# kcat/openal-soft

Hardware: NVIDIA H100
Metric: voice-samples/s mixed (HRTF, bsinc24, 1024-frame updates) (higher is better)
Workload: dtype f32

## Files before the change

openal-soft_b200/csrc/async_ptx.cuh:

```cuda
#pragma once
#include <cstdint>
#include <cuda_runtime.h>

namespace b200mix {

__device__ __forceinline__ uint32_t smem_u32(const void *p)
{ return static_cast<uint32_t>(__cvta_generic_to_shared(p)); }

__device__ __forceinline__ void mbar_init(uint64_t *bar, uint32_t count)
{ asm volatile("mbarrier.init.shared::cta.b64 [%0], %1;" :: "r"(smem_u32(bar)), "r"(count) : "memory"); }
__device__ __forceinline__ void mbar_fence_init()
{ asm volatile("fence.mbarrier_init.release.cluster;" ::: "memory"); }
__device__ __forceinline__ void mbar_expect_tx(uint64_t *bar, uint32_t bytes)
{ asm volatile("mbarrier.arrive.expect_tx.shared::cta.b64 _, [%0], %1;" :: "r"(smem_u32(bar)), "r"(bytes) : "memory"); }
__device__ __forceinline__ void mbar_arrive(uint64_t *bar)
{ asm volatile("mbarrier.arrive.shared::cta.b64 _, [%0];" :: "r"(smem_u32(bar)) : "memory"); }
__device__ __forceinline__ bool mbar_try_wait(uint64_t *bar, uint32_t parity)
{
    uint32_t ok;
    asm volatile("{\n\t.reg .pred p;\n\t"
                 "mbarrier.try_wait.parity.shared::cta.b64 p, [%1], %2;\n\t"
                 "selp.u32 %0, 1, 0, p;\n\t}"
                 : "=r"(ok) : "r"(smem_u32(bar)), "r"(parity) : "memory");
    return ok != 0u;
}
__device__ __forceinline__ void mbar_wait(uint64_t *bar, uint32_t parity)
{ while(!mbar_try_wait(bar, parity)) { } }

__device__ __forceinline__ void bulk_g2s(void *dst_smem, const void *src_gmem, uint32_t bytes, uint64_t *bar)
{
    asm volatile("cp.async.bulk.shared::cluster.global.mbarrier::complete_tx::bytes [%0], [%1], %2, [%3];"
        :: "r"(smem_u32(dst_smem)), "l"(src_gmem), "r"(bytes), "r"(smem_u32(bar)) : "memory");
}
__device__ __forceinline__ void fence_proxy_async_smem()
{ asm volatile("fence.proxy.async.shared::cta;" ::: "memory"); }

__device__ __forceinline__ uint64_t wgmma_smem_desc(uint32_t saddr, uint32_t lbo_bytes, uint32_t sbo_bytes)
{
    return uint64_t((saddr >> 4) & 0x3fffu) | (uint64_t((lbo_bytes >> 4) & 0x3fffu) << 16)
        | (uint64_t((sbo_bytes >> 4) & 0x3fffu) << 32);
}
__device__ __forceinline__ void wgmma_fence() { asm volatile("wgmma.fence.sync.aligned;" ::: "memory"); }
__device__ __forceinline__ void wgmma_commit() { asm volatile("wgmma.commit_group.sync.aligned;" ::: "memory"); }
template<int N> __device__ __forceinline__ void wgmma_wait()
{ asm volatile("wgmma.wait_group.sync.aligned %0;" :: "n"(N) : "memory"); }
__device__ __forceinline__ void wgmma_m64n16k8_tf32(float (&d)[8], uint64_t adesc, uint64_t bdesc, bool accumulate)
{
    asm volatile("{\n\t.reg .pred p;\n\tsetp.ne.b32 p, %10, 0;\n\t"
                 "wgmma.mma_async.sync.aligned.m64n16k8.f32.tf32.tf32 "
                 "{%0,%1,%2,%3,%4,%5,%6,%7}, %8, %9, p, 1, 1;\n\t}"
        : "+f"(d[0]), "+f"(d[1]), "+f"(d[2]), "+f"(d[3]), "+f"(d[4]), "+f"(d[5]), "+f"(d[6]), "+f"(d[7])
        : "l"(adesc), "l"(bdesc), "r"(uint32_t(accumulate)) : "memory");
}

}
```

openal-soft_b200/csrc/b200mix.cu:

```cuda
#include "../../include/b200mix.h"

#include <algorithm>
#include <cmath>
#include <cstdio>
#include <cstdlib>
#include <cstring>
#include <new>
#include <string>
#include <vector>

#include <cuda_runtime.h>

#include <dlfcn.h>

#include "mixer_kernels.cuh"
#include "effect_kernels.cuh"
#include "shard_kernels.cuh"
#include "panmix_tc.cuh"
#include "param_kernels.hpp"
#include "efx_kernels.hpp"
#include "resampler_tables.hpp"
#include "hrtf_store.hpp"
#include "adpcm.hpp"
#include "callback_plan.hpp"
// ... 3 lines not shown

namespace {

thread_local std::string g_create_error;

}

struct b200mix_device {
    b200mix_device_desc desc{};
    int cuda_dev{0};
    int num_sms{0};
    cudaStream_t stream{nullptr};
    std::string error;
    uint64_t launches{0};

    BsincTable bsinc[3];
    DevArray<float> d_bsinc[3], d_cubic[2];

    DevArray<VoiceRec> d_voices; DevArray<BufferRec> d_buffers;
    std::vector<BufferRec> h_buffers;
    std::vector<DevArray<char>> buf_store;
    std::vector<uint32_t> h_vbuf;
    std::vector<uint32_t> h_bufrefs;
    DevArray<float2> d_hrtf_tgt, d_hrtf_old;
    DevArray<float> d_dry_cur, d_dry_tgt, d_send_cur, d_send_tgt;
    VoiceResult *d_results{nullptr};
    b200mix_voice_result *h_results{nullptr};
    DevArray<char> d_outblock; PinnedArray<char> h_outblock; size_t out_real_bytes{0};

    uint32_t dry_alloc_ch{0};
    DevArray<float> d_dry, d_wet;
    float *d_real{nullptr};
    DevArray<float> d_partial; size_t partial_floats{0};
    DevArray<float> d_accum_sum;
    DevArray<float> d_carry[2];
    int carry_idx{0};
    float *h_real{nullptr};

    uint32_t dec_channels{0}, dec_ir{0};
    DevArray<float2> d_dec_coef; DevArray<float> d_dec_hfscale, d_dec_state;
    DevArray<float> d_temp, d_temp2;
    uint32_t amb_in{0}; bool amb_dual{false};
    DevArray<float> d_amb_hf, d_amb_lf, d_amb_state;
    bool dry_active{false};
    DevArray<float> d_uhj_state, d_uhj_scratch;
    uint32_t stab_center{B200MIX_NO_SLOT};
    float stab_coeff{0.0f};
    DevArray<float> d_stab_state;
    uint32_t bs2b_level{0};
    DevArray<float> d_bs2b;
    uint32_t uhj_fir{0};
    DevArray<float> d_uhj_fir_state, d_uhj_fir_coef;

    UploadArena stage;

    std::vector<SlotRec> h_slots;
    DevArray<SlotRec> d_slots;
    std::vector<std::vector<DevArray<char>>> slot_allocs;
    uint32_t active_slots{0};
    DevArray<float> d_xscratch; DevArray<uint32_t> d_sendinfo;
    DevArray<FilterRec> d_filt;
    UploadArena fstage;
    DevArray<float> d_fscratch, d_dline;
    std::vector<uint8_t> h_dfilt;
    std::vector<uint32_t> h_order2;
    DevArray<uint32_t> d_order2;
    uint32_t num_order2{0};
// ... 57 lines not shown
    std::vector<uint32_t> h_order;
    DevArray<uint32_t> d_order;
    uint32_t num_order{0};
    bool order_dirty{true};

    UploadArena src;
    bool dev_filters{false};
    bool panmix_tc{false};

    struct Shard {
        uint32_t rank{0}, world{1}; int transport{0};
        DevArray<char> own;
        char *peer[kShardMaxWorld]{};
        size_t off_real{0}, off_wet{0}, real_floats{0}, wet_src_floats{0};
        uint32_t owned_max{0};
        uint32_t epoch{0};
        DevArray<uint32_t> d_counters;
        PinnedArray<uint32_t> h_status;
        Event ev[4];
        bool ev_wet{false}, ev_real{false};
        void *nccl_lib{nullptr}; void *comm{nullptr};
        int (*reduce)(const void*, void*, size_t, int, int, int, void*, cudaStream_t){nullptr};
        int (*allreduce)(const void*, void*, size_t, int, int, void*, cudaStream_t){nullptr};
        int (*comm_destroy)(void*){nullptr};
    } shard;

    uint32_t ir_pad{0};
    uint32_t voice_hi{0};
    void (*mix_fn)(const MixParams){nullptr};
    size_t mix_smem{0}; int mix_cdr{0}; int mix_blocks_per_sm{1};
    uint32_t reverb_seq{0};
    DevArray<uint32_t> d_claim;
    int fir_blocks_per_sm{0};

    struct CbBuf {
        bool used{false};
        uint32_t buffer{0};
        b200mix_callback_buffer cb{};
        cbplan::State st{};
        uint32_t frame_bytes{0};
    };
    std::vector<CbBuf> cbs;
    std::vector<int32_t> cb_of_buffer;
    struct CbVoice { int32_t slot{-1}; cbplan::Voice v{}; };
    std::vector<CbVoice> cbv;
    uint32_t cb_bound{0};
    UploadArena cb_arena[2]; int cb_idx{0};
    DevArray<char> d_cb_zero;
    std::vector<int32_t> cb_reps;
    std::vector<std::vector<uint32_t>> cb_members;
    struct CbWork { cbplan::State start; cbplan::Loads loads; size_t region{0}, bytes{0}; };
    std::vector<CbWork> cb_work;
    ~b200mix_device() { if(stream) cudaStreamDestroy(stream); }
};

namespace {
constexpr uint32_t kCbMaxChannels = 16;
constexpr size_t kCbPad = 256;
}

namespace {

#define CUDA_TRY(dev, expr) do { cudaError_t e_ = (expr); if(e_ != cudaSuccess) {            \
    (dev)->error = std::string(#expr) + ": " + cudaGetErrorString(e_); return B200MIX_ERR_CUDA; } } while(0)

template<typename T>
int upload(b200mix_device *d, DevArray<T> &dst, const std::vector<T> &src)
{
    if(!src.empty())
        CUDA_TRY(d, cudaMemcpyAsync(dst.get(), src.data(), src.size()*sizeof(T), cudaMemcpyHostToDevice, d->stream));
    CUDA_TRY(d, cudaStreamSynchronize(d->stream));
    return B200MIX_OK;
}

using MixKernel = void(*)(const MixParams);

struct FirVariant { MixKernel fn; size_t smem; };
FirVariant get_fir(uint32_t ir_size)
{
    if(ir_size <= 64u)
        return FirVariant{k_hrtf_fir<17, 64>, sizeof(FirSmem<kFirGS, 17, 64>)*kFirGroups};
    return FirVariant{k_hrtf_fir<19, 128>, sizeof(FirSmem<kFirGS, 19, 128>)*kFirGroups};
}

constexpr uint32_t kDryChunksMax = 128;

int ensure_park_lines(b200mix_device *d)
{
    if(d->d_xscratch) return B200MIX_OK;
    const uint32_t nv = d->desc.max_voices;
    DevArray<float> xscratch; DevArray<uint32_t> sendinfo;
    CUDA_TRY(d, xscratch.alloc(size_t(nv)*kLine, d->stream));
    CUDA_TRY(d, sendinfo.alloc(nv, d->stream));
    d->d_xscratch = std::move(xscratch); d->d_sendinfo = std::move(sendinfo);
    return B200MIX_OK;
}

int ensure_dry_park(b200mix_device *d)
{
    const b200mix_device_desc &dd = d->desc;
    if(d->d_dry_entries) return B200MIX_OK;
    if(int rc = ensure_park_lines(d)) return rc;
    if(dd.dry_channels > 4u && dd.dry_channels <= uint32_t(kPmN))
    {
        CUDA_TRY(d, cudaFuncSetAttribute(k_panmix_tc, cudaFuncAttributeMaxDynamicSharedMemorySize,
            kPmStages*kPmStageBytes + 1024));
        const char *simt = std::getenv("B200MIX_PANMIX_SIMT");
        d->panmix_tc = !(simt && simt[0] == '1');
    }
    DevArray<SendEntry> entries; DevArray<uint32_t> slotStart;
    DevArray<float> partial, geff; DevArray<float4> gramp;
    CUDA_TRY(d, entries.alloc(dd.max_voices, d->stream));
    CUDA_TRY(d, slotStart.alloc(2, d->stream));
    CUDA_TRY(d, partial.alloc(size_t(kDryChunksMax)*dd.dry_channels*kLine, d->stream));
    CUDA_TRY(d, geff.alloc(size_t(dd.max_voices)*dd.dry_channels, d->stream));
    CUDA_TRY(d, gramp.alloc(size_t(dd.max_voices)*dd.dry_channels, d->stream));
    d->d_dry_entries = std::move(entries); d->d_dry_slot_start = std::move(slotStart);
// ... 154 lines not shown
        {
            if(int rc = ensure_park_lines(d)) return rc;
            CUDA_TRY(d, d->d_claim.alloc(2, d->stream));
        }
        if(hrtfDev)
        {
            const FirVariant fir = get_fir(dd.ir_size);
            CUDA_TRY(d, cudaFuncSetAttribute(fir.fn, cudaFuncAttributeMaxDynamicSharedMemorySize, int(fir.smem)));
            CUDA_TRY(d, cudaOccupancyMaxActiveBlocksPerMultiprocessor(&perSm, fir.fn, kFirGS*kFirGroups, fir.smem));
            d->fir_blocks_per_sm = std::max(std::min(perSm, kFirCtasPerSm), 1);
        }

        d->dry_alloc_ch = std::max<uint32_t>(std::max(dd.dry_channels, 1u), uint32_t(d->mix_cdr));
        CUDA_TRY(d, d->d_dry.alloc(size_t(d->dry_alloc_ch)*kLine, d->stream));
        {
            const size_t realFloats = size_t(std::max(dd.real_channels, 1u))*kLine;
            static_assert(sizeof(VoiceResult) == 16 && sizeof(b200mix_voice_result) == 16, "result layout");
            const size_t blockBytes = realFloats*sizeof(float) + size_t(dd.max_voices)*sizeof(VoiceResult);
            CUDA_TRY(d, d->d_outblock.alloc(blockBytes, d->stream));
            char *blk = d->d_outblock;
            d->d_results = reinterpret_cast<VoiceResult*>(blk + realFloats*sizeof(float));
            CUDA_TRY(d, d->h_outblock.alloc(blockBytes));
            d->h_real = reinterpret_cast<float*>(d->h_outblock.get());
            d->h_results = reinterpret_cast<b200mix_voice_result*>(d->h_outblock + realFloats*sizeof(float));
            d->out_real_bytes = realFloats*sizeof(float);
            if(dd.post_process == B200MIX_POST_NONE) d->d_real = d->d_dry;
            else d->d_real = reinterpret_cast<float*>(blk);
        }
        if(dd.max_slots && dd.wet_channels)
            CUDA_TRY(d, d->d_wet.alloc(size_t(dd.max_slots)*dd.wet_channels*kLine, d->stream));
        d->partial_floats = hrtfDev ? size_t(d->num_sms)*d->fir_blocks_per_sm*(2*kAccumLen)
            : size_t(d->num_sms)*d->mix_blocks_per_sm*size_t(d->mix_cdr)*kLine;
        CUDA_TRY(d, d->d_partial.alloc(std::max<size_t>((hrtfDev ? 1 : 2)*d->partial_floats, 4), d->stream));
        CUDA_TRY(d, d->d_accum_sum.alloc(2*kAccumLen, d->stream));
        CUDA_TRY(d, d->d_carry[0].alloc(2*kHrirLen, d->stream));
        CUDA_TRY(d, d->d_carry[1].alloc(2*kHrirLen, d->stream));
        CUDA_TRY(d, d->d_temp.alloc(size_t(std::max(dd.dry_channels, 1u))*kLine, d->stream));
        CUDA_TRY(d, d->d_temp2.alloc(size_t(std::max(dd.dry_channels, 1u))*kLine, d->stream));
        if(dd.max_slots && dd.wet_channels && dd.num_sends)
        {
            d->h_slots.assign(dd.max_slots, SlotRec{});
            d->slot_allocs.resize(dd.max_slots);
            CUDA_TRY(d, d->d_slots.alloc(dd.max_slots, d->stream));
            if(int rc = ensure_park_lines(d)) return rc;
            CUDA_TRY(d, d->d_send_geff.alloc(size_t(dd.max_voices)*dd.num_sends*dd.wet_channels, d->stream));
            CUDA_TRY(d, d->d_send_gramp.alloc(size_t(dd.max_voices)*dd.num_sends*dd.wet_channels, d->stream));
            d->h_send_slot.assign(size_t(dd.max_voices)*B200MIX_MAX_SENDS, B200MIX_NO_SLOT);
            CUDA_TRY(d, d->d_slot_start.alloc(dd.max_slots + 1, d->stream));
            CUDA_TRY(d, d->d_entries.alloc(size_t(dd.max_voices)*dd.num_sends, d->stream));
            std::vector<float2> tw(128);
            for(int k = 0;k < 128;++k)
            {
                const double a = -2.0*3.14159265358979323846*double(k)/256.0;
                tw[k] = make_float2(float(std::cos(a)), float(std::sin(a)));
            }
            const std::vector<float> cf = BuildCubicFilter();
            CUDA_TRY(d, d->d_cubic_filter.alloc(cf.size()));
            if(int rc = upload(d, d->d_cubic_filter, cf)) return rc;
            CUDA_TRY(d, d->d_twiddle.alloc(tw.size()));
            if(int rc = upload(d, d->d_twiddle, tw)) return rc;
        }
        if(dd.post_process == B200MIX_POST_UHJ || dd.post_process == B200MIX_POST_TSME)
        {
            CUDA_TRY(d, d->d_uhj_state.alloc(64, d->stream));
            CUDA_TRY(d, d->d_uhj_scratch.alloc(5*1025, d->stream));
        }
        if(int rc = ensure_stage(d, std::min(dd.max_voices, 4096u))) return rc;
// ... 1338 lines not shown
        for(uint32_t v : d->h_order) if(d->dev_filters || d->h_dfilt[v]) d->h_order2.push_back(v);
        d->num_order2 = uint32_t(d->h_order2.size());
        if(d->num_order2)
            if(int rc = upload(d, d->d_order2, d->h_order2)) return rc;
        d->order2_dirty = false;
    }
    const bool hrtfDev = dd.ir_size > 0;
    const uint32_t nv = std::max(d->voice_hi, 1u);
    const uint32_t maxBlocks = uint32_t(d->num_sms*d->mix_blocks_per_sm);
    const uint32_t blocks = std::max(1u, std::min(maxBlocks, (d->num_order + kMixGroups - 1)/kMixGroups));

    MixParams P{};
    P.voices = d->d_voices; P.buffers = d->d_buffers;
    P.hrtf_tgt = d->d_hrtf_tgt; P.hrtf_old = d->d_hrtf_old;
    P.dry_cur = d->d_dry_cur; P.dry_tgt = d->d_dry_tgt;
    P.partial = d->d_partial;
    P.results = want_results ? d->d_results : nullptr;
    for(int i = 0;i < 3;++i) P.bsinc_tab[i] = d->d_bsinc[i];
    for(int i = 0;i < 2;++i) P.cubic_tab[i] = d->d_cubic[i];
    P.max_voices = nv; P.frames = frames; P.ir_pad = d->ir_pad;
    P.cd = dd.dry_channels; P.num_sends = dd.num_sends;
    P.order = d->d_order; P.num_order = d->num_order;
    P.xscratch = d->d_xscratch; P.sendinfo = d->d_sendinfo;
    P.filt = d->d_filt; P.filt_paths = 1u + dd.num_sends;
    P.qhdr = d->d_qhdr; P.queue = d->d_queue;
    P.claim = d->d_claim;
    P.dline = d->d_dline;
    P.cbplan = cbplan;
    stage_mark(d, 1);
    if(d->profile) cudaEventRecord(d->ev_mix0, d->stream);
    d->mix_fn<<<blocks, kMixGS*kMixGroups, d->mix_smem, d->stream>>>(P);
    ++d->launches;
    CUDA_TRY(d, cudaGetLastError());

    stage_mark(d, 2);
    size_t rows2 = 0;
    if(d->d_filt && d->num_order2)
    {
        FilterRunParams FP{};
        FP.filt = d->d_filt; FP.filt_paths = 1u + dd.num_sends; FP.sendinfo = d->d_sendinfo;
        FP.direct_order = d->d_order2; FP.num_direct = d->num_order2;
        FP.xscratch = d->d_xscratch; FP.dline = d->d_dline; FP.frames = frames;
        k_filters<<<(d->num_order2 + 31u)/32u, 32, 0, d->stream>>>(FP);
        ++d->launches;
        if(d->mix_cdr > 0)
        {
            const uint32_t blocks2 = std::max(1u, std::min(maxBlocks, (d->num_order2 + kMixGroups - 1)/kMixGroups));
            rows2 = blocks2;
            MixParams P2 = P;
            P2.order = d->d_order2; P2.num_order = d->num_order2;
            P2.partial = d->d_partial + d->partial_floats;
            P2.results = nullptr;
            k_mix_deferred<kMixGS, kMixGroups, 4><<<blocks2, kMixGS*kMixGroups,
                sizeof(DeferredSmem<kMixGroups, 4>), d->stream>>>(P2);
            ++d->launches;
        }
        CUDA_TRY(d, cudaGetLastError());
    }
    uint32_t firBlocks = 0;
    if(hrtfDev)
    {
        const FirVariant fir = get_fir(dd.ir_size);
        firBlocks = std::max(1u, std::min(uint32_t(d->num_sms*d->fir_blocks_per_sm),
            (d->num_order + kFirGroups - 1)/kFirGroups));
        fir.fn<<<firBlocks, kFirGS*kFirGroups, fir.smem, d->stream>>>(P);
        ++d->launches;
        CUDA_TRY(d, cudaGetLastError());
    }
    if(d->profile) { cudaEventRecord(d->ev_mix1, d->stream); d->ev_valid = true; }

    stage_mark(d, 3);
    if(hrtfDev)
    {
        const uint32_t len = 2*kAccumLen;
        k_reduce_rows<<<(len/4 + kReduceCols - 1)/kReduceCols, 1024, 0, d->stream>>>(d->d_partial, firBlocks, len,
            d->d_accum_sum, 0);
        ++d->launches;
    }
    if(d->mix_cdr > 0)
    {
        const uint32_t len = uint32_t(d->mix_cdr)*kLine;
        k_reduce_rows<<<(len/4 + kReduceCols - 1)/kReduceCols, 1024, 0, d->stream>>>(d->d_partial, blocks, len, d->d_dry, 1);
        ++d->launches;
        if(rows2)
        {
            k_reduce_rows<<<(len/4 + kReduceCols - 1)/kReduceCols, 1024, 0, d->stream>>>(d->d_partial + d->partial_floats,
                uint32_t(rows2), len, d->d_dry, 1);
            ++d->launches;
        }
    }
    CUDA_TRY(d, cudaGetLastError());

    stage_mark(d, 4);
    if(d->mix_cdr == 0 && d->d_dry_entries)
    {
        if(d->dry_entries_dirty)
        {
            d->h_dry_entries.clear();
            for(uint32_t v = 0;v < d->voice_hi;++v)
                if(d->h_active[v] && !d->h_hrtf[v]) d->h_dry_entries.push_back(SendEntry{v, 0u});
            d->num_dry_entries = uint32_t(d->h_dry_entries.size());
            const uint32_t ss[2] = {0u, d->num_dry_entries};
            CUDA_TRY(d, cudaMemcpyAsync(d->d_dry_slot_start, ss, sizeof(ss), cudaMemcpyHostToDevice, d->stream));
            if(int rc = upload(d, d->d_dry_entries, d->h_dry_entries)) return rc;
            d->dry_entries_dirty = false;
        }
        if(d->num_dry_entries)
        {
            SendMixParams DM{};
            DM.slot_start = d->d_dry_slot_start; DM.entries = d->d_dry_entries; DM.sendinfo = d->d_sendinfo;
            DM.xscratch = d->d_xscratch; DM.send_cur = d->d_dry_cur; DM.send_tgt = d->d_dry_tgt;
// ... 152 lines not shown
            }
            if(convWork)
            {
                k_conv_input<<<dd.max_slots, 128, 0, d->stream>>>(CP);
                k_conv_mac<<<dim3(dd.max_slots, convCh, CP.chunks), 128, sizeof(ConvMacSmem), d->stream>>>(CP);
                k_conv_ifft<<<dim3(dd.max_slots, convCh, kConvMaxBlocks), 128, 0, d->stream>>>(CP);
                k_conv_output<<<dim3(dd.max_slots, convCh), 128, 0, d->stream>>>(CP);
                d->launches += 4;
            }
            k_slot_output_mix<<<dim3((frames + 127)/128, dd.dry_channels), 128, 0, d->stream>>>(SP);
            ++d->launches;
            if(d->any_target)
            {
                k_slot_target_mix<<<dim3((frames + 127)/128, dd.max_slots), 128, 0, d->stream>>>(SP);
                ++d->launches;
            }
        }
        k_slot_gains_commit<<<dd.max_slots, 64, 0, d->stream>>>(SP);
        ++d->launches;
        for(auto &eh : d->efx)
        {
            if(eh.used && eh.p.type == B200MIX_EFFECT_MODULATOR) eh.mod_index = (eh.mod_index + frames) % eh.mod_range;
            if(eh.used && eh.p.type == B200MIX_EFFECT_CHORUS) eh.lfo_offset = (eh.lfo_offset + frames) % eh.lfo_range;
        }
        CUDA_TRY(d, cudaGetLastError());
    }

    stage_mark(d, 7);
    switch(dd.post_process)
    {
    case B200MIX_POST_HRTF:
    {
        PostHrtfParams Q{};
        Q.accum_sum = d->d_accum_sum; Q.carry_in = d->d_carry[d->carry_idx];
        Q.carry_out = d->d_carry[d->carry_idx^1];
        Q.dry = d->d_dry; Q.real = d->d_real; Q.dec_coef = d->d_dec_coef;
        Q.dec_hfscale = d->d_dec_hfscale; Q.dec_state = d->d_dec_state; Q.temp = d->d_temp;
        Q.frames = frames; Q.cd = dd.dry_channels; Q.dec_ir = d->dec_ir;
        Q.real_left = dd.real_left; Q.real_right = dd.real_right; Q.dry_active = d->dry_active;
        if(d->dry_active)
        {
            k_post_hrtf_split<<<dd.dry_channels, 32, 0, d->stream>>>(Q);
            ++d->launches;
        }
        Q.overwrite = d->real_overwrite ? 1u : 0u;
        k_post_hrtf_mix<<<dim3((frames + kHrirLen + 127)/128, 2), 128, 0, d->stream>>>(Q);
        ++d->launches;
        d->carry_idx ^= 1;
        break;
    }
    case B200MIX_POST_AMBIDEC:
    {
        PostAmbiParams Q{};
        Q.dry = d->d_dry; Q.real = d->d_real; Q.gains_hf = d->d_amb_hf; Q.gains_lf = d->d_amb_lf;
        Q.split_state = d->d_amb_state; Q.temp_hf = d->d_temp; Q.temp_lf = d->d_temp2;
        Q.frames = frames; Q.cd = dd.dry_channels; Q.real_channels = dd.real_channels;
        Q.dual = d->amb_dual;
        if(d->amb_dual)
        {
            k_post_ambi_split<<<1, 32, 0, d->stream>>>(Q);
            ++d->launches;
        }
        const uint32_t total = dd.real_channels*frames;
        k_post_ambi_mix<<<(total + 127)/128, 128, 0, d->stream>>>(Q);
        ++d->launches;
        if(d->stab_center != B200MIX_NO_SLOT)
        {
            StabParams S{};
            S.real = d->d_real; S.state = d->d_stab_state; S.frames = frames;
            S.real_channels = dd.real_channels; S.lidx = dd.real_left; S.ridx = dd.real_right;
            S.cidx = d->stab_center; S.coeff = d->stab_coeff;
            const float halfPi = 3.14159265358979323846f*0.5f;
            S.mid_lf = std::cos(1.0f/3.0f * halfPi); S.mid_hf = std::cos(1.0f/4.0f * halfPi);
            S.center_lf = std::sin(1.0f/3.0f * halfPi); S.center_hf = std::sin(1.0f/4.0f * halfPi);
            const size_t smem = size_t(2u + dd.real_channels)*kLine*sizeof(float);
            k_post_stabilizer<<<1, 32u*dd.real_channels, smem, d->stream>>>(S);
            ++d->launches;
        }
        else if(d->bs2b_level)
        {
// ... 29 lines not shown
}

static int render_output_stage(b200mix_device *d, uint32_t frames)
{
    const b200mix_device_desc &dd = d->desc;
    if(d->shard.transport && d->shard.rank != 0u) return B200MIX_OK;
    if(d->d_limiter)
    {
        LimiterParams LQ{d->d_limiter, d->d_real, d->d_limiter_delay, frames};
        k_limiter<<<1, 1024, 0, d->stream>>>(LQ);
        ++d->launches;
    }
    if(d->d_dc_delay)
    {
        DistCompParams DQ{d->d_real, d->d_dc_buf, d->d_dc_delay, d->d_dc_gain, frames};
        k_distance_comp<<<dd.real_channels, 1024, 0, d->stream>>>(DQ);
        ++d->launches;
    }
    CUDA_TRY(d, cudaGetLastError());
    return B200MIX_OK;
}

static int shard_wet_exchange(b200mix_device *d)
{
    b200mix_device::Shard &S = d->shard;
    const b200mix_device_desc &dd = d->desc;
    if(!S.transport || !d->d_wet) return B200MIX_OK;
    if(d->profile) { cudaEventRecord(S.ev[0], d->stream); }
    const size_t wetFloats = size_t(dd.max_slots)*dd.wet_channels*kLine;
    if(S.transport == 2)
    {
        if(S.allreduce(d->d_wet, d->d_wet, wetFloats, 7 , 0 , S.comm, d->stream) != 0)
        { d->error = "ncclAllReduce of the wet buffers failed"; return B200MIX_ERR_CUDA; }
    }
    else
    {
        const uint32_t slotFloats = dd.wet_channels*uint32_t(kLine);
        ShardPushParams P{};
        P.src = d->d_wet; P.rank = S.rank; P.world = S.world; P.epoch = S.epoch;
        P.wet = 1u; P.num_slots = dd.max_slots; P.slot_floats = slotFloats; P.owned_max = S.owned_max;
        P.own = reinterpret_cast<ShardCtl*>(S.own.get());
        for(uint32_t r = 0;r < S.world;++r) P.peer[r] = S.peer[r];
        P.off_data = S.off_wet; P.per_src_floats = S.wet_src_floats;
        P.counters = S.d_counters + 4;
        const uint32_t chunks = std::max(1u, std::min(32u, slotFloats*S.owned_max/(4u*256u*4u)));
        k_shard_push<<<dim3(chunks, S.world), 256, 0, d->stream>>>(P);
        ShardSumParams Q{};
        Q.dst = d->d_wet; Q.rank = S.rank; Q.world = S.world; Q.epoch = S.epoch;
        Q.wet = 1u; Q.num_slots = dd.max_slots; Q.slot_floats = slotFloats; Q.owned_max = S.owned_max;
        Q.own = P.own; for(uint32_t r = 0;r < S.world;++r) Q.peer[r] = S.peer[r];
        Q.off_data = S.off_wet; Q.per_src_floats = S.wet_src_floats; Q.counter = S.d_counters + 2;
        k_shard_sum<<<std::max(1u, std::min(64u, slotFloats*S.owned_max/(4u*256u*2u))), 256, 0, d->stream>>>(Q);
        d->launches += 2;
        CUDA_TRY(d, cudaGetLastError());
    }
    if(d->profile) { cudaEventRecord(S.ev[1], d->stream); S.ev_wet = true; }
    return B200MIX_OK;
}

static int shard_real_reduce(b200mix_device *d)
{
    b200mix_device::Shard &S = d->shard;
    const b200mix_device_desc &dd = d->desc;
    if(!S.transport) return B200MIX_OK;
    if(d->profile) { cudaEventRecord(S.ev[2], d->stream); }
    const uint32_t floats = dd.real_channels*uint32_t(kLine);
// ... 280 lines not shown
        || (dither_depth > 0.0f && !dither_seed))
    { d->error = "render_interleaved: bad arguments"; return B200MIX_ERR_INVALID; }
    if(int rc = render_launch(d, frames, results != nullptr)) return rc;
    static const size_t sz[] = {1, 1, 2, 2, 4, 4, 4};
    if(!d->h_outbuf)
    {
        CUDA_TRY(d, d->d_outbuf.alloc(size_t(kLine)*64*4));
        CUDA_TRY(d, d->h_outbuf.alloc(size_t(kLine)*64*4));
    }
    OutputParams Q{};
    Q.real = d->d_real; Q.out = d->d_outbuf; Q.frames = frames; Q.channels = dd.real_channels;
    Q.frame_step = frame_step; Q.out_type = out_type; Q.dither_depth = dither_depth;
    Q.seed = dither_seed ? *dither_seed : 0u;
    const uint32_t total = frames*frame_step;
    k_output_write<<<(total + 255)/256, 256, 0, d->stream>>>(Q);
    ++d->launches;
    CUDA_TRY(d, cudaGetLastError());
    const size_t bytes = size_t(total)*sz[out_type];
    CUDA_TRY(d, cudaMemcpyAsync(d->h_outbuf, d->d_outbuf, bytes, cudaMemcpyDeviceToHost, d->stream));
    if(int rc = render_collect(d, frames, nullptr, results)) return rc;
    std::memcpy(out, d->h_outbuf, bytes);
    if(dither_depth > 0.0f) *dither_seed = lcg_skip_host(*dither_seed, uint64_t(2)*dd.real_channels*frames);
    return B200MIX_OK;
}

int b200mix_render_begin(b200mix_device *d, uint32_t frames, float **wet_dev, size_t *wet_floats)
{
    if(!d) return B200MIX_ERR_INVALID;
    if(d->mid_render) { d->error = "render_begin: already begun"; return B200MIX_ERR_INVALID; }
    if(d->shard.transport)
    { d->error = "render_begin: a sharded device set exchanges its wet buffers itself — use b200mix_render"; return B200MIX_ERR_INVALID; }
    if(int rc = render_phase_a(d, frames, true, true)) return rc;
    d->mid_render = true; d->mid_frames = frames;
    if(wet_dev) *wet_dev = d->d_wet;
    if(wet_floats) *wet_floats = d->d_wet ? size_t(d->desc.max_slots)*d->desc.wet_channels*kLine : 0;
    return B200MIX_OK;
}

int b200mix_render_end(b200mix_device *d, float *const *real_out, b200mix_voice_result *results,
    const float **real_out_dev)
{
    if(!d) return B200MIX_ERR_INVALID;
    if(!d->mid_render) { d->error = "render_end: no render_begin pending"; return B200MIX_ERR_INVALID; }
    d->mid_render = false;
    if(int rc = render_phase_b(d, d->mid_frames)) return rc;
    if(int rc = render_output_stage(d, d->mid_frames)) return rc;
    if(real_out_dev) *real_out_dev = d->d_real;
    if(!real_out && !results) return B200MIX_OK;
    return render_collect(d, d->mid_frames, real_out, results);
}

int b200mix_render_device(b200mix_device *d, uint32_t frames, const float **real_out_dev)
{
    if(!d) return B200MIX_ERR_INVALID;
    if(int rc = render_launch(d, frames, false)) return rc;
    if(real_out_dev) *real_out_dev = d->d_real;
    return B200MIX_OK;
}

static void shard_release(b200mix_device *d)
{
    b200mix_device::Shard &S = d->shard;
    if(S.transport == 1)
        for(uint32_t r = 0;r < S.world;++r)
            if(r != S.rank && S.peer[r]) cudaIpcCloseMemHandle(S.peer[r]);
    if(S.comm && S.comm_destroy) S.comm_destroy(S.comm);
// ... 212 lines not shown
```

openal-soft_b200/csrc/mixer_kernels.cuh:

```cuda
#pragma once
#include <cstddef>
#include <cstdint>
#include <cuda_runtime.h>

#include "voice_structs.hpp"
#include "async_ptx.cuh"

namespace b200mix {

constexpr int kLine = 1024;
constexpr int kHrirLen = 128;
constexpr int kHist = 64;
constexpr int kEdge = 24;
constexpr int kPad = 48;
constexpr int kResBuf = kLine + 256 + kPad;
constexpr int kSrcSizeMax = kResBuf - kEdge;
constexpr int kAccumLen = kLine + kHrirLen;
constexpr float kSilence = 0.00001f;
constexpr float kEps = 1.1920929e-07f;

constexpr uint32_t kVfStatic = 1u<<2, kVfLooping = 1u<<3, kVfHrtf = 1u<<4;
constexpr uint32_t kVfFading = 1u<<8, kVfHaveBuffer = 1u<<9, kVfCoefDirty = 1u<<10;
constexpr uint32_t kUpNoBuffer = 1u<<11;
constexpr uint32_t kVfChannelMask = 0xffu<<16;
// ... 1015 lines not shown
                }
                group_sync(bar, GS);

                if(pack && winInt && !packedWin)
                {
                    pack_window16<GS>(S.win, srcn, t, bar);
                    packedWin = true;
                }
                resample_chunk<GS>(S.win, S.tabF, S.tabD, xs, loaded, dstn, increment, fracPos,
                    resampler, m, tapOff, ms, packedWin, t);
            }
            advance_chunk<GS>(S.win, rec.prev, packedWin, silent, playing, n, loaded, dstn, increment,
                fracPos, intPos, t, bar);
        }
        group_sync(bar, GS);

        const uint32_t counter = (flags & kVfFading) ? (n < 64u ? n : 64u) : 0u;
        if(P.sendinfo)
            park_voice<GS, CDR>(P, xs, v, rec.send_mask, defer, isHrtf, playing, dirty, counter, t);
        if(dfilt && !defer) filter_clear(*dfilt, t);
        if constexpr(CDR > 0)
            if(!defer)
                mix_dry<GS, CDR>(accD, xs, S.newGain, P.dry_cur + size_t(v)*P.cd, P.dry_tgt + size_t(v)*P.cd,
                    P.cd, n, counter, playing, t);
        if(t == 0)
            write_back_voice(P, rec, v, h1, flags, vstate, increment, haveBuffer, isQueue, qh, qitems,
                looping, loopStart, loopEnd, buf.frames);
        group_sync(bar, GS);
        if(CDR > 0 && !defer) store_dry_gains(P.dry_cur + size_t(v)*P.cd, S.newGain, P.cd, t);
        group_sync(bar, GS);
    }

    if constexpr(CDR > 0) store_partial_row<GS, GROUPS, CDR>(accD, smem_raw, P.partial, g, t);
}

template<int GROUPS, int CDR>
union DeferredSmem {
    struct { float x[kLine]; float newGain[32]; } group[GROUPS];
    float stage[CDR*kLine];
};

template<int GS, int GROUPS, int CDR>
__global__ void __launch_bounds__(GS*GROUPS)
k_mix_deferred(const MixParams P)
{
    extern __shared__ __align__(16) unsigned char smem_raw[];
    const int g = threadIdx.x / GS;
    const int t = threadIdx.x % GS;
    auto &S = reinterpret_cast<DeferredSmem<GROUPS, CDR>*>(smem_raw)->group[g];
    const int bar = 1 + g;
    constexpr int SPT = kLine / GS;

    float accD[CDR][SPT];
    #pragma unroll
    for(int c = 0;c < CDR;++c)
        #pragma unroll
        for(int r = 0;r < SPT;++r) accD[c][r] = 0.0f;

    const uint32_t n = P.frames;
    const uint32_t groups = gridDim.x*GROUPS;
    for(uint32_t oi = blockIdx.x*GROUPS + g;oi < P.num_order;oi += groups)
    {
        const uint32_t v = P.order[oi];
        const uint32_t info = P.sendinfo[v];
        if(!(info & kSiDeferred)) continue;
        const float *fl = P.dline + size_t(v)*kLine;
// ... 28 lines not shown
    const uint32_t lineBytes = (n & ~3u)*4u, irBytes = P.ir_pad*8u;
    const bool dirty = (info & kSiDirty) != 0;
    const float *line = ((info & kSiDeferred) ? P.dline : P.xscratch) + size_t(v)*kLine;
    fence_proxy_async_smem();
    mbar_expect_tx(bar, kHist*4u + lineBytes + (dirty ? 2u : 1u)*irBytes);
    bulk_g2s(B.x, P.voices[v].hist, kHist*4u, bar);
    if(lineBytes) bulk_g2s(B.x + kHist, line, lineBytes, bar);
    bulk_g2s(B.coefT, P.hrtf_tgt + size_t(v)*P.ir_pad, irBytes, bar);
    if(dirty) bulk_g2s(B.coefO, P.hrtf_old + size_t(v)*P.ir_pad, irBytes, bar);
}

template<int OPT, int FP>
__global__ void __launch_bounds__(kFirGS*kFirGroups, kFirCtasPerSm)
k_hrtf_fir(const MixParams P)
{
    constexpr int GS = kFirGS, GROUPS = kFirGroups;
    using Smem = FirSmem<GS, OPT, FP>;
    extern __shared__ __align__(16) unsigned char smem_raw[];
    const int g = threadIdx.x / GS;
    const int t = threadIdx.x % GS;
    Smem &S = reinterpret_cast<Smem*>(smem_raw)[g];
    const int bar = 1 + g;
    const int t0 = OPT*t;
    const uint32_t n = P.frames;

    float2 acc[OPT];
    #pragma unroll
    for(int r = 0;r < OPT;++r) acc[r] = make_float2(0.0f, 0.0f);

    for(int i = t;i < FP;i += GS) S.lLR[i] = make_float2(0.0f, 0.0f);
    for(int i = FP + int(n) + t;i < Smem::kLLen;i += GS) S.lLR[i] = make_float2(0.0f, 0.0f);
    if(t == 0) { mbar_init(&S.bar[0], 1u); mbar_init(&S.bar[1], 1u); mbar_fence_init(); }
    group_sync(bar, GS);

    const uint32_t stride = gridDim.x*GROUPS;
    uint32_t v = 0u, info = 0u;
    uint32_t oi = next_hrtf_voice(P, blockIdx.x*GROUPS + g, stride, v, info);
    if(t == 0 && oi < P.num_order) fir_stage_issue(P, S.st[0], &S.bar[0], v, info, n);
    uint32_t parity = 0u;
    for(int b = 0;oi < P.num_order;b ^= 1)
    {
        VoiceRec &rec = P.voices[v];
        const uint4 *hp = reinterpret_cast<const uint4*>(&rec);
        const uint4 h3 = hp[3], h4 = hp[4];

        uint32_t vN = 0u, infoN = 0u;
        const uint32_t oiN = next_hrtf_voice(P, oi + stride, stride, vN, infoN);
        if(t == 0 && oiN < P.num_order) fir_stage_issue(P, S.st[b^1], &S.bar[b^1], vN, infoN, n);

        FirStage &B = S.st[b];
        const bool playing = (info & kSiPlaying) != 0;
        const bool dirty = (info & kSiDirty) != 0;
        const uint32_t counter = (info >> 8) & 0xffu;

        const float *line = ((info & kSiDeferred) ? P.dline : P.xscratch) + size_t(v)*kLine;
        for(uint32_t k = (n & ~3u) + t;k < n;k += GS) B.x[kHist + k] = line[k];
        mbar_wait(&S.bar[b], (parity >> b) & 1u);
        parity ^= 1u << b;
        if(n & 3u) group_sync(bar, GS);

        if(playing)
            for(int k = t;k < kHist;k += GS) rec.hist[k] = B.x[n + k];
        uint32_t oD0 = h4.x, oD1 = h4.y;
        float oGain = __uint_as_float(h4.z);
        const uint32_t tD0 = h3.y, tD1 = h3.z;
        const float tgtGain = __uint_as_float(h3.w);
// ... 38 lines not shown
            in[s] = make_float2(xl[s] * gnew, xr[s] * gnew);
        }
        const bool oldPass = !sameFilter && oldOn;
        if(oldPass)
            for(int i = t;i < Smem::kOLen;i += GS)
            {
                const int s = i - FP;
                float l = 0.0f, r = 0.0f;
                if(s >= 0 && uint32_t(s) < fademix)
                {
                    const float gold = oldStep*float(fademix - uint32_t(s));
                    l = hs[kHist - oD0 + s] * gold;
                    r = hs[kHist - oD1 + s] * gold;
                }
                S.oLR[i] = make_float2(l, r);
            }
        group_sync(bar, GS);

        const int irpad = int(P.ir_pad);
        fir_pass<OPT, FP>(acc, S.lLR, B.coefT, irpad, t0);
        if(oldPass && t0 < int(kHist) + irpad)
            fir_pass<OPT, FP>(acc, S.oLR, dirty ? B.coefO : B.coefT, irpad, t0);
        if(t == 0)
        {
            rec.old_delay0 = tD0; rec.old_delay1 = tD1;
            rec.old_gain = targetGain;
        }
        group_sync(bar, GS);
        oi = oiN; v = vN; info = infoN;
    }

    const size_t row = blockIdx.x;
    __syncthreads();
    float *stage = reinterpret_cast<float*>(smem_raw);
    for(int gg = 0;gg < GROUPS;++gg)
    {
        if(g == gg)
        {
            #pragma unroll
            for(int r = 0;r < OPT;++r)
            {
                const int o = t0 + r;
                if(o < kAccumLen)
                {
                    if(gg == 0) { stage[o] = acc[r].x; stage[kAccumLen + o] = acc[r].y; }
                    else { stage[o] += acc[r].x; stage[kAccumLen + o] += acc[r].y; }
                }
            }
            if(gg == 0 && GS*OPT < kAccumLen)
                for(int o = GS*OPT + t;o < kAccumLen;o += GS) { stage[o] = 0.0f; stage[kAccumLen + o] = 0.0f; }
        }
        __syncthreads();
    }
    float *pl = P.partial + row*(2*kAccumLen);
    for(int o = threadIdx.x;o < 2*kAccumLen;o += GS*GROUPS) pl[o] = stage[o];
}


constexpr int kReduceCols = 8, kReduceSegs = 128;
__global__ void __launch_bounds__(1024)
k_reduce_rows(const float *__restrict__ partial, uint32_t rows, uint32_t len,
    float *__restrict__ out, int accumulate)
{
    __shared__ float4 sm[kReduceSegs][kReduceCols];
    const uint32_t col = threadIdx.x & (kReduceCols-1), seg = threadIdx.x / kReduceCols;
    const uint32_t e4 = blockIdx.x*kReduceCols + col;
    float4 s = make_float4(0.f, 0.f, 0.f, 0.f);
    if(e4*4u < len)
    {
        const uint32_t per = (rows + kReduceSegs - 1u)/kReduceSegs;
        const uint32_t r0 = seg*per, r1 = (r0 + per < rows) ? r0 + per : rows;
        const float4 *p = reinterpret_cast<const float4*>(partial) + e4;
        const size_t stride4 = len/4u;
        uint32_t r = r0;
        for(;r + 4u <= r1;r += 4u)
        {
            const float4 a = __ldg(p + size_t(r)*stride4), b = __ldg(p + size_t(r+1)*stride4);
            const float4 c = __ldg(p + size_t(r+2)*stride4), d = __ldg(p + size_t(r+3)*stride4);
            s.x += a.x; s.y += a.y; s.z += a.z; s.w += a.w;
            s.x += b.x; s.y += b.y; s.z += b.z; s.w += b.w;
            s.x += c.x; s.y += c.y; s.z += c.z; s.w += c.w;
            s.x += d.x; s.y += d.y; s.z += d.z; s.w += d.w;
        }
        for(;r < r1;++r)
        {
            const float4 a = __ldg(p + size_t(r)*stride4);
            s.x += a.x; s.y += a.y; s.z += a.z; s.w += a.w;
        }
    }
    sm[seg][col] = s;
    __syncthreads();
    #pragma unroll
    for(uint32_t width = kReduceSegs/4u;width >= 1u;width /= 4u)
    {
        float4 tot = make_float4(0.f, 0.f, 0.f, 0.f);
        const bool on = seg < width;
        if(on)
        {
            tot = sm[seg*4u][col];
            #pragma unroll
            for(uint32_t k = 1;k < 4u;++k)
            {
                const float4 a = sm[seg*4u + k][col];
                tot.x += a.x; tot.y += a.y; tot.z += a.z; tot.w += a.w;
            }
        }
        __syncthreads();
        if(on) sm[seg][col] = tot;
        __syncthreads();
        if(width == 2u) break;
    }
    if(seg == 0 && e4*4u < len)
    {
        float4 tot = sm[0][col];
        const float4 b = sm[1][col];
        tot.x += b.x; tot.y += b.y; tot.z += b.z; tot.w += b.w;
        float4 *o = reinterpret_cast<float4*>(out) + e4;
        if(accumulate)
        {
            const float4 a = *o;
            tot.x += a.x; tot.y += a.y; tot.z += a.z; tot.w += a.w;
        }
        *o = tot;
    }
}

__global__ void __launch_bounds__(256)
k_reduce_few(const float *__restrict__ partial, uint32_t rows, uint32_t len,
    float *__restrict__ out, int accumulate)
{
    const uint32_t e4 = blockIdx.x*blockDim.x + threadIdx.x;
    if(e4*4u >= len) return;
    const float4 *p = reinterpret_cast<const float4*>(partial) + e4;
    const size_t stride4 = len/4u;
    float4 v[16];
    #pragma unroll
    for(uint32_t r = 0;r < 16u;++r)
        v[r] = r < rows ? __ldg(p + size_t(r)*stride4) : make_float4(0.f, 0.f, 0.f, 0.f);
    float4 g[4];
    #pragma unroll
    for(uint32_t j = 0;j < 4u;++j)
    {
        float4 t = v[4u*j];
        #pragma unroll
        for(uint32_t k = 1;k < 4u;++k)
        { t.x += v[4u*j+k].x; t.y += v[4u*j+k].y; t.z += v[4u*j+k].z; t.w += v[4u*j+k].w; }
        g[j] = t;
    }
    float4 tot = g[0];
// ... 216 lines not shown
            fl |= kVfHaveBuffer;
            if(up.flags & (1u<<6)) fl |= kVfFading;
            rec.old_delay0 = 0; rec.old_delay1 = 0; rec.old_gain = 0.0f;
            if(A.qhdr) A.qhdr[up.voice].y = 0u;
        }
        else
        {
            fl |= oldFlags & (kVfFading|kVfHaveBuffer|kVfCoefDirty);
        }
        if(up.has_coeffs && !reset) fl |= kVfCoefDirty;
        if(up.flags & kUpNoBuffer) fl &= ~kVfHaveBuffer;
        rec.flags = fl;
        if(up.flags & (1u<<7)) rec.state = 0u;
        else if(up.flags & (1u<<1)) rec.state = 2u;
        else if(up.flags & (1u<<0)) rec.state = 1u;
        rec.buffer = up.buffer; rec.resampler = up.resampler;
        rec.loop_start = up.loop_start; rec.loop_end = up.loop_end; rec.step = up.step;
        rec.bsinc_sf = up.bsinc_sf; rec.bsinc_m = up.bsinc_m; rec.bsinc_l = up.bsinc_l;
        rec.bsinc_off = up.bsinc_off;
        rec.tgt_delay0 = fromDirs ? sB.delay[0] : up.delay0;
        rec.tgt_delay1 = fromDirs ? sB.delay[1] : up.delay1;
        rec.tgt_gain = up.gain;
        uint32_t mask = 0;
        for(int s = 0;s < kMaxSends;++s)
        {
            rec.send_slot[s] = up.send_slot[s];
            if(up.send_slot[s] != 0xffffffffu) mask |= 1u<<s;
        }
        rec.send_mask = mask;
    }
}

struct PostHrtfParams {
    const float *accum_sum;
    const float *carry_in;
    float *carry_out;
    const float *dry;
    float *real;
    const float2 *dec_coef;
    const float *dec_hfscale; float *dec_state;
    float *temp;
    uint32_t frames, cd, dec_ir, real_left, real_right, dry_active;
    uint32_t overwrite;
};

__global__ void __launch_bounds__(32) k_post_hrtf_split(const PostHrtfParams Q)
{
    __shared__ float line[kLine];
    const uint32_t c = blockIdx.x;
    if(c >= Q.cd) return;
    const uint32_t lane = threadIdx.x, n = Q.frames;
    const float *in = Q.dry + size_t(c)*kLine;
    float *out = Q.temp + size_t(c)*kLine;
    for(uint32_t i = lane;i < kLine;i += 32) line[i] = (i < n) ? in[i] : 0.0f;
    __syncwarp();
    if(lane == 0)
    {
        float *st = Q.dec_state + c*4;
        const float ap_coeff = st[0];
        const float lp_coeff = st[0]*0.5f + 0.5f;
        float lp_z1 = st[1], lp_z2 = st[2], ap_z1 = st[3];
        const float hfscale = Q.dec_hfscale[c];
        for(uint32_t i0 = 0;i0 < n;i0 += 8)
        {
            float x[8], y[8];
            #pragma unroll
            for(int k = 0;k < 8;++k) x[k] = line[i0+k];
            #pragma unroll
            for(int k = 0;k < 8;++k)
            {
                const float d0 = (x[k] - lp_z1) * lp_coeff;
                const float lp_y0 = lp_z1 + d0;
                const float nz1 = lp_y0 + d0*lp_coeff;
                const float d1 = (lp_y0 - lp_z2) * lp_coeff;
                const float lp_y1 = lp_z2 + d1;
                const float nz2 = lp_y1 + d1;
                const float ap_y = x[k]*ap_coeff + ap_z1;
                const float naz = x[k] - ap_y*ap_coeff;
                y[k] = (ap_y-lp_y1)*hfscale + lp_y1;
                if(i0 + k < n) { lp_z1 = nz1; lp_z2 = nz2; ap_z1 = naz; }
            }
            #pragma unroll
            for(int k = 0;k < 8;++k) line[i0+k] = y[k];
        }
        st[1] = lp_z1; st[2] = lp_z2; st[3] = ap_z1;
    }
    __syncwarp();
    for(uint32_t i = lane;i < n;i += 32) out[i] = line[i];
}

__global__ void __launch_bounds__(128) k_post_hrtf_mix(const PostHrtfParams Q)
{
    __shared__ float xs[128 + kHrirLen];
    __shared__ float cf[kHrirLen];
    const uint32_t span = Q.frames + kHrirLen;
    const uint32_t ear = blockIdx.y;
    const uint32_t t0 = blockIdx.x*128u, tt = t0 + threadIdx.x;
    float tot = 0.0f;
    if(tt < span)
    {
        tot = Q.accum_sum[ear*kAccumLen + tt];
        if(tt < uint32_t(kHrirLen)) tot += Q.carry_in[ear*kHrirLen + tt];
    }
    if(Q.dry_active)
    {
        const uint32_t jmax = Q.dec_ir;
        for(uint32_t c = 0;c < Q.cd;++c)
        {
            const float *x = Q.temp + size_t(c)*kLine;
            const float2 *cg = Q.dec_coef + size_t(c)*Q.dec_ir;
            __syncthreads();
            for(uint32_t k = threadIdx.x;k < 128u + kHrirLen;k += 128u)
            {
                const int src = int(t0) - int(kHrirLen) + int(k);
                xs[k] = (src >= 0 && src < int(Q.frames)) ? x[src] : 0.0f;
            }
            if(threadIdx.x < jmax) cf[threadIdx.x] = ear ? cg[threadIdx.x].y : cg[threadIdx.x].x;
            __syncthreads();
            float s = 0.0f;
            const float *w = xs + kHrirLen + threadIdx.x;
            for(uint32_t j = 0;j < jmax;++j)
                s = fmaf(cf[j], w[-int(j)], s);
            tot += s;
        }
    }
    if(tt >= span) return;
    if(tt < Q.frames)
    {
        float *o = Q.real + size_t(ear ? Q.real_right : Q.real_left)*kLine + tt;
        *o = Q.overwrite ? tot : (*o + tot);
    }
    else
        Q.carry_out[ear*kHrirLen + (tt - Q.frames)] = tot;
}

struct PostAmbiParams {
    const float *dry; float *real; const float *gains_hf; const float *gains_lf;
    float *split_state; float *temp_hf; float *temp_lf;
    uint32_t frames, cd, real_channels, dual;
};

__global__ void k_post_ambi_split(const PostAmbiParams Q)
{
    const uint32_t c = blockIdx.x*blockDim.x + threadIdx.x;
    if(c >= Q.cd) return;
    float *st = Q.split_state + c*4;
    const float ap_coeff = st[0];
    const float lp_coeff = st[0]*0.5f + 0.5f;
    float lp_z1 = st[1], lp_z2 = st[2], ap_z1 = st[3];
    const float *in = Q.dry + size_t(c)*kLine;
    float *hp = Q.temp_hf + size_t(c)*kLine, *lp = Q.temp_lf + size_t(c)*kLine;
    for(uint32_t i = 0;i < Q.frames;++i)
    {
        const float x = in[i];
        const float d0 = (x - lp_z1) * lp_coeff;
        const float lp_y0 = lp_z1 + d0;
        lp_z1 = lp_y0 + d0;
        const float d1 = (lp_y0 - lp_z2) * lp_coeff;
        const float lp_y1 = lp_z2 + d1;
        lp_z2 = lp_y1 + d1;
        lp[i] = lp_y1;
        const float ap_y = x*ap_coeff + ap_z1;
        ap_z1 = x - ap_y*ap_coeff;
// ... 677 lines not shown
```

Baseline: 31.06 billion.

## Fuse HRTF partial-row reduction into post-HRTF mix and chain kernels with PDL

Removes the separate k_reduce_rows launch and the accum_sum buffer by having a new k_post_hrtf_reduce kernel sum FIR partial rows per 32-sample tile, then add the carry and the per-channel decoder FIR, with one thread per (dry channel, output). Adds programmatic dependent launch (griddepcontrol) between the mix, FIR and post kernels so each can start its prologue before the previous one finishes. The reduce loop is also batched eight rows at a time to keep more loads in flight. In exchange, many more blocks each re-read decoder coefficients and input, and the post kernel is limited to 32 dry channels.

After: 32.29 billion, median of 6. 1.04x the previous value.

```diff
diff --git a/openal-soft_b200/csrc/async_ptx.cuh b/openal-soft_b200/csrc/async_ptx.cuh
--- a/openal-soft_b200/csrc/async_ptx.cuh
+++ b/openal-soft_b200/csrc/async_ptx.cuh
@@ -35,6 +35,10 @@
 __device__ __forceinline__ void fence_proxy_async_smem()
 { asm volatile("fence.proxy.async.shared::cta;" ::: "memory"); }
 
+__device__ __forceinline__ void griddep_wait() { asm volatile("griddepcontrol.wait;" ::: "memory"); }
+__device__ __forceinline__ void griddep_launch_dependents()
+{ asm volatile("griddepcontrol.launch_dependents;" ::: "memory"); }
+
 __device__ __forceinline__ uint64_t wgmma_smem_desc(uint32_t saddr, uint32_t lbo_bytes, uint32_t sbo_bytes)
 {
     return uint64_t((saddr >> 4) & 0x3fffu) | (uint64_t((lbo_bytes >> 4) & 0x3fffu) << 16)
diff --git a/openal-soft_b200/csrc/b200mix.cu b/openal-soft_b200/csrc/b200mix.cu
--- a/openal-soft_b200/csrc/b200mix.cu
+++ b/openal-soft_b200/csrc/b200mix.cu
@@ -59,7 +59,7 @@
     DevArray<float> d_dry, d_wet;
     float *d_real{nullptr};
     DevArray<float> d_partial; size_t partial_floats{0};
-    DevArray<float> d_accum_sum;
+    uint32_t fir_rows{0};
     DevArray<float> d_carry[2];
     int carry_idx{0};
     float *h_real{nullptr};
@@ -183,6 +183,7 @@
     uint32_t reverb_seq{0};
     DevArray<uint32_t> d_claim;
     int fir_blocks_per_sm{0};
+    uint64_t fir_done{0};
 
     struct CbBuf {
         bool used{false};
@@ -234,6 +235,22 @@
     return FirVariant{k_hrtf_fir<19, 128>, sizeof(FirSmem<kFirGS, 19, 128>)*kFirGroups};
 }
 
+static_assert(kPostMaxDry == B200MIX_MAX_DRY_CHANNELS, "k_post_hrtf_reduce: one thread per dry channel");
+
+template<typename... Args>
+cudaError_t launch_ex(b200mix_device *d, bool programmatic, void (*fn)(Args...), dim3 grid, dim3 block,
+    size_t smem, Args... args)
+{
+    cudaLaunchAttribute attr{};
+    attr.id = cudaLaunchAttributeProgrammaticStreamSerialization;
+    attr.val.programmaticStreamSerializationAllowed = 1;
+    cudaLaunchConfig_t cfg{};
+    cfg.gridDim = grid; cfg.blockDim = block; cfg.dynamicSmemBytes = smem; cfg.stream = d->stream;
+    cfg.attrs = programmatic ? &attr : nullptr; cfg.numAttrs = programmatic ? 1u : 0u;
+    ++d->launches;
+    return cudaLaunchKernelEx(&cfg, fn, args...);
+}
+
 constexpr uint32_t kDryChunksMax = 128;
 
 int ensure_park_lines(b200mix_device *d)
@@ -454,7 +471,6 @@
         d->partial_floats = hrtfDev ? size_t(d->num_sms)*d->fir_blocks_per_sm*(2*kAccumLen)
             : size_t(d->num_sms)*d->mix_blocks_per_sm*size_t(d->mix_cdr)*kLine;
         CUDA_TRY(d, d->d_partial.alloc(std::max<size_t>((hrtfDev ? 1 : 2)*d->partial_floats, 4), d->stream));
-        CUDA_TRY(d, d->d_accum_sum.alloc(2*kAccumLen, d->stream));
         CUDA_TRY(d, d->d_carry[0].alloc(2*kHrirLen, d->stream));
         CUDA_TRY(d, d->d_carry[1].alloc(2*kHrirLen, d->stream));
         CUDA_TRY(d, d->d_temp.alloc(size_t(std::max(dd.dry_channels, 1u))*kLine, d->stream));
@@ -1859,6 +1875,7 @@
     d->mix_fn<<<blocks, kMixGS*kMixGroups, d->mix_smem, d->stream>>>(P);
     ++d->launches;
     CUDA_TRY(d, cudaGetLastError());
+    const uint64_t mixDone = d->launches;
 
     stage_mark(d, 2);
     size_t rows2 = 0;
@@ -1884,26 +1901,19 @@
         }
         CUDA_TRY(d, cudaGetLastError());
     }
-    uint32_t firBlocks = 0;
+    d->fir_rows = 0;
     if(hrtfDev)
     {
         const FirVariant fir = get_fir(dd.ir_size);
-        firBlocks = std::max(1u, std::min(uint32_t(d->num_sms*d->fir_blocks_per_sm),
+        d->fir_rows = std::max(1u, std::min(uint32_t(d->num_sms*d->fir_blocks_per_sm),
             (d->num_order + kFirGroups - 1)/kFirGroups));
-        fir.fn<<<firBlocks, kFirGS*kFirGroups, fir.smem, d->stream>>>(P);
-        ++d->launches;
-        CUDA_TRY(d, cudaGetLastError());
+        CUDA_TRY(d, launch_ex(d, d->launches == mixDone, fir.fn, dim3(d->fir_rows), dim3(kFirGS*kFirGroups),
+            fir.smem, P));
+        d->fir_done = d->launches;
     }
     if(d->profile) { cudaEventRecord(d->ev_mix1, d->stream); d->ev_valid = true; }
 
     stage_mark(d, 3);
-    if(hrtfDev)
-    {
-        const uint32_t len = 2*kAccumLen;
-        k_reduce_rows<<<(len/4 + kReduceCols - 1)/kReduceCols, 1024, 0, d->stream>>>(d->d_partial, firBlocks, len,
-            d->d_accum_sum, 0);
-        ++d->launches;
-    }
     if(d->mix_cdr > 0)
     {
         const uint32_t len = uint32_t(d->mix_cdr)*kLine;
@@ -2122,7 +2132,7 @@
     case B200MIX_POST_HRTF:
     {
         PostHrtfParams Q{};
-        Q.accum_sum = d->d_accum_sum; Q.carry_in = d->d_carry[d->carry_idx];
+        Q.partial = d->d_partial; Q.rows = d->fir_rows; Q.carry_in = d->d_carry[d->carry_idx];
         Q.carry_out = d->d_carry[d->carry_idx^1];
         Q.dry = d->d_dry; Q.real = d->d_real; Q.dec_coef = d->d_dec_coef;
         Q.dec_hfscale = d->d_dec_hfscale; Q.dec_state = d->d_dec_state; Q.temp = d->d_temp;
@@ -2134,8 +2144,8 @@
             ++d->launches;
         }
         Q.overwrite = d->real_overwrite ? 1u : 0u;
-        k_post_hrtf_mix<<<dim3((frames + kHrirLen + 127)/128, 2), 128, 0, d->stream>>>(Q);
-        ++d->launches;
+        CUDA_TRY(d, launch_ex(d, d->launches == d->fir_done, k_post_hrtf_reduce,
+            dim3((frames + kHrirLen + kPostTile - 1)/kPostTile, 2), dim3(1024), 0, Q));
         d->carry_idx ^= 1;
         break;
     }
@@ -2231,6 +2241,7 @@
     {
         if(S.allreduce(d->d_wet, d->d_wet, wetFloats, 7 , 0 , S.comm, d->stream) != 0)
         { d->error = "ncclAllReduce of the wet buffers failed"; return B200MIX_ERR_CUDA; }
+        d->fir_done = 0;
     }
     else
     {
@@ -2577,6 +2588,7 @@
     { d->error = "render_begin: a sharded device set exchanges its wet buffers itself — use b200mix_render"; return B200MIX_ERR_INVALID; }
     if(int rc = render_phase_a(d, frames, true, true)) return rc;
     d->mid_render = true; d->mid_frames = frames;
+    d->fir_done = 0;
     if(wet_dev) *wet_dev = d->d_wet;
     if(wet_floats) *wet_floats = d->d_wet ? size_t(d->desc.max_slots)*d->desc.wet_channels*kLine : 0;
     return B200MIX_OK;
diff --git a/openal-soft_b200/csrc/mixer_kernels.cuh b/openal-soft_b200/csrc/mixer_kernels.cuh
--- a/openal-soft_b200/csrc/mixer_kernels.cuh
+++ b/openal-soft_b200/csrc/mixer_kernels.cuh
@@ -1071,6 +1071,11 @@
     }
 
     if constexpr(CDR > 0) store_partial_row<GS, GROUPS, CDR>(accD, smem_raw, P.partial, g, t);
+    else
+    {
+        __syncthreads();
+        griddep_launch_dependents();
+    }
 }
 
 template<int GROUPS, int CDR>
@@ -1165,6 +1170,7 @@
     for(int i = FP + int(n) + t;i < Smem::kLLen;i += GS) S.lLR[i] = make_float2(0.0f, 0.0f);
     if(t == 0) { mbar_init(&S.bar[0], 1u); mbar_init(&S.bar[1], 1u); mbar_fence_init(); }
     group_sync(bar, GS);
+    griddep_wait();
 
     const uint32_t stride = gridDim.x*GROUPS;
     uint32_t v = 0u, info = 0u;
@@ -1269,6 +1275,7 @@
 
     const size_t row = blockIdx.x;
     __syncthreads();
+    griddep_launch_dependents();
     float *stage = reinterpret_cast<float*>(smem_raw);
     for(int gg = 0;gg < GROUPS;++gg)
     {
@@ -1295,34 +1302,28 @@
 
 
 constexpr int kReduceCols = 8, kReduceSegs = 128;
-__global__ void __launch_bounds__(1024)
-k_reduce_rows(const float *__restrict__ partial, uint32_t rows, uint32_t len,
-    float *__restrict__ out, int accumulate)
-{
-    __shared__ float4 sm[kReduceSegs][kReduceCols];
+
+__device__ __forceinline__ float4 reduce_rows_cta(const float *__restrict__ partial, uint32_t rows,
+    uint32_t len, uint32_t e4, bool live, float4 (&sm)[kReduceSegs][kReduceCols])
+{
     const uint32_t col = threadIdx.x & (kReduceCols-1), seg = threadIdx.x / kReduceCols;
-    const uint32_t e4 = blockIdx.x*kReduceCols + col;
     float4 s = make_float4(0.f, 0.f, 0.f, 0.f);
-    if(e4*4u < len)
+    if(live)
     {
         const uint32_t per = (rows + kReduceSegs - 1u)/kReduceSegs;
         const uint32_t r0 = seg*per, r1 = (r0 + per < rows) ? r0 + per : rows;
         const float4 *p = reinterpret_cast<const float4*>(partial) + e4;
         const size_t stride4 = len/4u;
-        uint32_t r = r0;
-        for(;r + 4u <= r1;r += 4u)
-        {
-            const float4 a = __ldg(p + size_t(r)*stride4), b = __ldg(p + size_t(r+1)*stride4);
-            const float4 c = __ldg(p + size_t(r+2)*stride4), d = __ldg(p + size_t(r+3)*stride4);
-            s.x += a.x; s.y += a.y; s.z += a.z; s.w += a.w;
-            s.x += b.x; s.y += b.y; s.z += b.z; s.w += b.w;
-            s.x += c.x; s.y += c.y; s.z += c.z; s.w += c.w;
-            s.x += d.x; s.y += d.y; s.z += d.z; s.w += d.w;
-        }
-        for(;r < r1;++r)
-        {
-            const float4 a = __ldg(p + size_t(r)*stride4);
-            s.x += a.x; s.y += a.y; s.z += a.z; s.w += a.w;
+        constexpr uint32_t kBatch = 8;
+        for(uint32_t r = r0;r < r1;r += kBatch)
+        {
+            float4 a[kBatch];
+            #pragma unroll
+            for(uint32_t k = 0;k < kBatch;++k)
+                if(r + k < r1) a[k] = __ldg(p + size_t(r + k)*stride4);
+            #pragma unroll
+            for(uint32_t k = 0;k < kBatch;++k)
+                if(r + k < r1) { s.x += a[k].x; s.y += a[k].y; s.z += a[k].z; s.w += a[k].w; }
         }
     }
     sm[seg][col] = s;
@@ -1347,11 +1348,25 @@
         __syncthreads();
         if(width == 2u) break;
     }
-    if(seg == 0 && e4*4u < len)
-    {
-        float4 tot = sm[0][col];
+    float4 tot = make_float4(0.f, 0.f, 0.f, 0.f);
+    if(seg == 0)
+    {
+        tot = sm[0][col];
         const float4 b = sm[1][col];
         tot.x += b.x; tot.y += b.y; tot.z += b.z; tot.w += b.w;
+    }
+    return tot;
+}
+
+__global__ void __launch_bounds__(1024)
+k_reduce_rows(const float *__restrict__ partial, uint32_t rows, uint32_t len,
+    float *__restrict__ out, int accumulate)
+{
+    __shared__ float4 sm[kReduceSegs][kReduceCols];
+    const uint32_t e4 = blockIdx.x*kReduceCols + (threadIdx.x & (kReduceCols-1));
+    float4 tot = reduce_rows_cta(partial, rows, len, e4, e4*4u < len, sm);
+    if(threadIdx.x < kReduceCols && e4*4u < len)
+    {
         float4 *o = reinterpret_cast<float4*>(out) + e4;
         if(accumulate)
         {
@@ -1634,7 +1649,8 @@
 }
 
 struct PostHrtfParams {
-    const float *accum_sum;
+    const float *partial;
+    uint32_t rows;
     const float *carry_in;
     float *carry_out;
     const float *dry;
@@ -1691,46 +1707,49 @@
     for(uint32_t i = lane;i < n;i += 32) out[i] = line[i];
 }
 
-__global__ void __launch_bounds__(128) k_post_hrtf_mix(const PostHrtfParams Q)
-{
-    __shared__ float xs[128 + kHrirLen];
-    __shared__ float cf[kHrirLen];
+constexpr uint32_t kPostTile = kReduceCols*4u, kPostMaxDry = 32u;
+static_assert(kAccumLen % kPostTile == 0, "a tile lies within one ear's accumulator");
+static_assert(kPostMaxDry*kPostTile <= 1024u, "one thread per (channel, output)");
+__global__ void __launch_bounds__(1024, 1) k_post_hrtf_reduce(const PostHrtfParams Q)
+{
+    __shared__ float4 sm[kReduceSegs][kReduceCols];
+    __shared__ float vsum[kPostTile];
+    __shared__ float dsum[kPostMaxDry][kPostTile];
     const uint32_t span = Q.frames + kHrirLen;
     const uint32_t ear = blockIdx.y;
-    const uint32_t t0 = blockIdx.x*128u, tt = t0 + threadIdx.x;
-    float tot = 0.0f;
-    if(tt < span)
-    {
-        tot = Q.accum_sum[ear*kAccumLen + tt];
-        if(tt < uint32_t(kHrirLen)) tot += Q.carry_in[ear*kHrirLen + tt];
-    }
+    const uint32_t t0 = blockIdx.x*kPostTile;
+    griddep_wait();
+    const uint32_t col = threadIdx.x & (kReduceCols-1);
+    const uint32_t e4 = (ear*kAccumLen + t0)/4u + col;
+    const float4 v = reduce_rows_cta(Q.partial, Q.rows, 2u*kAccumLen, e4, t0 + 4u*col < span, sm);
+    if(threadIdx.x < kReduceCols)
+    { vsum[4*col] = v.x; vsum[4*col + 1] = v.y; vsum[4*col + 2] = v.z; vsum[4*col + 3] = v.w; }
+
+    const uint32_t o = threadIdx.x % kPostTile, c = threadIdx.x / kPostTile;
+    const uint32_t tt = t0 + o;
+    if(Q.dry_active && c < Q.cd)
+    {
+        const float *x = Q.temp + size_t(c)*kLine;
+        const float2 *cg = Q.dec_coef + size_t(c)*Q.dec_ir;
+        float s = 0.0f;
+        for(uint32_t j = 0;j < Q.dec_ir;++j)
+        {
+            const int src = int(tt) - int(j);
+            const float xv = (src >= 0 && src < int(Q.frames)) ? x[src] : 0.0f;
+            s = fmaf(ear ? cg[j].y : cg[j].x, xv, s);
+        }
+        dsum[c][o] = s;
+    }
+    __syncthreads();
+    if(threadIdx.x >= kPostTile || tt >= span) return;
+    float tot = vsum[o];
+    if(tt < uint32_t(kHrirLen)) tot += Q.carry_in[ear*kHrirLen + tt];
     if(Q.dry_active)
-    {
-        const uint32_t jmax = Q.dec_ir;
-        for(uint32_t c = 0;c < Q.cd;++c)
-        {
-            const float *x = Q.temp + size_t(c)*kLine;
-            const float2 *cg = Q.dec_coef + size_t(c)*Q.dec_ir;
-            __syncthreads();
-            for(uint32_t k = threadIdx.x;k < 128u + kHrirLen;k += 128u)
-            {
-                const int src = int(t0) - int(kHrirLen) + int(k);
-                xs[k] = (src >= 0 && src < int(Q.frames)) ? x[src] : 0.0f;
-            }
-            if(threadIdx.x < jmax) cf[threadIdx.x] = ear ? cg[threadIdx.x].y : cg[threadIdx.x].x;
-            __syncthreads();
-            float s = 0.0f;
-            const float *w = xs + kHrirLen + threadIdx.x;
-            for(uint32_t j = 0;j < jmax;++j)
-                s = fmaf(cf[j], w[-int(j)], s);
-            tot += s;
-        }
-    }
-    if(tt >= span) return;
+        for(uint32_t ch = 0;ch < Q.cd;++ch) tot += dsum[ch][o];
     if(tt < Q.frames)
     {
-        float *o = Q.real + size_t(ear ? Q.real_right : Q.real_left)*kLine + tt;
-        *o = Q.overwrite ? tot : (*o + tot);
+        float *out = Q.real + size_t(ear ? Q.real_right : Q.real_left)*kLine + tt;
+        *out = Q.overwrite ? tot : (*out + tot);
     }
     else
         Q.carry_out[ear*kHrirLen + (tt - Q.frames)] = tot;
```
